# balkce/beamform

Hardware: AMD Instinct MI355X
Metric: stft_frames_per_sec (higher is better)
Workload: dtype f64; 1 GPU; das 8-mic 1024-pt (hop 512), 65536-frame batch per GPU, 1 stream(s), planar input resident in HBM; frames_per_gpu=65536, frames_fed_per_gpu=65536, mics=8, fft=1024, hop=512, streams=1, layout=planar, gather=n/a, parallelism=independent batches x1, input=uniform noise in [-0.5, 0.5), settle_launches_before_warmup=416, forward_transforms_per_frame_pair=6

## Files before the change

beamform_amd/csrc/das_f64_w64.hip:

```cpp
#include <hip/hip_runtime.h>

#include <cstdlib>
#include <cstring>
#include <type_traits>

#include "launch_trace.hpp"
#include "das_f64_plan.hpp"
#include "pipeline_kernels.hpp"
#include "w64_f64_dev.hpp"

namespace bf {

namespace {

constexpr int kBlock = 512;
constexpr int kWaves = kBlock / 64;
constexpr int kHop = 512;
constexpr int kTwD = 2 * (1024 + 4 * kTw2RowW64Rot);
constexpr int oTw = 0;
constexpr int oPlane = kTwD;
constexpr int oGain = oPlane + kWaves * kPlaneD;
constexpr int oCross = oGain + 4 * 2048;
constexpr int oFlag = oCross + 512;
constexpr int kWinRow = 18;
constexpr int oWin = oFlag + 8;
constexpr int kLdsD = oWin + 64 * kWinRow;

typedef volatile __attribute__((address_space(3))) int *lds_flag_t;

template <int LAYOUT>
__global__ __launch_bounds__(kBlock) void das_f64_w64_kernel(DasF64Args a, int frames_per_chunk, int chunks_per_stream) {
    __shared__ __attribute__((aligned(16))) double lds[kLdsD];
    const cx<double> *s_tw1 = reinterpret_cast<const cx<double> *>(lds + oTw);
    const cx<double> *s_tw2 = s_tw1 + 1024;
    const cx<double> *s_gain = reinterpret_cast<const cx<double> *>(lds + oGain);
    float *s_cross = reinterpret_cast<float *>(lds + oCross);
    lds_flag_t s_ready = (lds_flag_t)(lds + oFlag);
    lds_flag_t s_cons = s_ready + kWaves;

    const int tid = threadIdx.x, lane = tid & 63;
    const int w = __builtin_amdgcn_readfirstlane(tid >> 6);
    const int M = a.n_mics, NP = (M + 1) >> 1;
    double *plane = lds + oPlane + w * kPlaneD;
    double *wcol = plane + w64_col_rot(lane);
    double *row16 = plane + (lane & 15) * kRS + 16 * (lane >> 4);

    const int stream = blockIdx.x / chunks_per_stream;
    const long c_in_s = blockIdx.x - (long)stream * chunks_per_stream;
    const double *wrow = lds + oWin + lane * kWinRow;

    const long T0 = c_in_s * frames_per_chunk;
    long T1 = T0 + frames_per_chunk;
    if (T1 > a.n_frames) T1 = a.n_frames;
    const float *xs = a.x + (long)stream * a.stream_stride_x;
    const float *hs = a.hist + (long)stream * M * kHop;
    float *ys = a.y + (long)stream * a.n_frames * kHop;

    float na[16], nb[16];
    auto request = [&](long tt, int p) {
        const int ma = 2 * p, mb = (2 * p + 1 < M) ? 2 * p + 1 : ma;
        if (LAYOUT == 0) {
            const float *a1 = tt >= 1 ? xs + (long)ma * a.mic_stride + (tt - 1) * kHop : hs + ma * kHop;
            const float *b1 = tt >= 1 ? xs + (long)mb * a.mic_stride + (tt - 1) * kHop : hs + mb * kHop;
            const float *a2 = xs + (long)ma * a.mic_stride + tt * kHop;
            const float *b2 = xs + (long)mb * a.mic_stride + tt * kHop;
#pragma unroll
            for (int j = 0; j < 8; ++j) {
                na[j] = a1[(unsigned)(64 * j + lane)];
                nb[j] = b1[(unsigned)(64 * j + lane)];
                na[j + 8] = a2[(unsigned)(64 * j + lane)];
                nb[j + 8] = b2[(unsigned)(64 * j + lane)];
            }
        } else {
            const float *s1 = tt >= 1 ? xs + (tt - 1) * (long)kHop * M : hs;
            const float *s2 = xs + tt * (long)kHop * M;
            if ((M & 1) == 0) {
#pragma unroll
                for (int j = 0; j < 8; ++j) {
                    const float2 v1 = *reinterpret_cast<const float2 *>(s1 + (unsigned)((64 * j + lane) * M + ma));
                    const float2 v2 = *reinterpret_cast<const float2 *>(s2 + (unsigned)((64 * j + lane) * M + ma));
                    na[j] = v1.x;
                    nb[j] = v1.y;
                    na[j + 8] = v2.x;
                    nb[j + 8] = v2.y;
                }
            } else {
#pragma unroll
                for (int j = 0; j < 8; ++j) {
                    na[j] = s1[(unsigned)((64 * j + lane) * M + ma)];
                    nb[j] = s1[(unsigned)((64 * j + lane) * M + mb)];
                    na[j + 8] = s2[(unsigned)((64 * j + lane) * M + ma)];
                    nb[j + 8] = s2[(unsigned)((64 * j + lane) * M + mb)];
                }
            }
        }
    };

    const int n_iter = (int)((T1 - T0 + kWaves - 1) / kWaves);
    if (T0 + w < T1) request(T0 + w, 0);
    {
        const f64x2 *tw2 = a.tw, *g2 = a.gains;
        f64x2 *ltw = reinterpret_cast<f64x2 *>(lds + oTw), *lg = reinterpret_cast<f64x2 *>(lds + oGain);
#pragma unroll 4
        for (int i = tid; i < kTwD / 2; i += kBlock) ltw[i] = tw2[i];
#pragma unroll 8
        for (int i = tid; i < NP * 1024; i += kBlock) lg[i] = g2[i];
#pragma unroll 2
        for (int i = tid; i < 1024; i += kBlock) lds[oWin + (i & 63) * kWinRow + (i >> 6)] = a.win[i];
        if (tid < 2 * kWaves) s_ready[tid] = -2;
    }
    __syncthreads();
    for (int it = 0; it < n_iter; ++it) {
        const long t = T0 + (long)it * kWaves + w;
        if (t >= T1) break;

        double Sr[16], Si[16];
        for (int p = 0; p < NP; ++p) {
            double re[16], im[16];
            const bool b_ok = 2 * p + 1 < M;
#pragma unroll
            for (int j = 0; j < 8; ++j) {
                const double w0 = wrow[j], w1 = wrow[j + 8];
                const double t = (double)na[j] * w0, u = (double)na[j + 8];
                re[j] = fma(u, w1, t);
                re[j + 8] = fma(-u, w1, t);
            }
            if (b_ok) {
#pragma unroll
                for (int j = 0; j < 8; ++j) {
                    const double w0 = wrow[j], w1 = wrow[j + 8];
                    const double t = (double)nb[j] * w0, u = (double)nb[j + 8];
                    im[j] = fma(u, w1, t);
                    im[j + 8] = fma(-u, w1, t);
                }
            } else {
#pragma unroll
                for (int j = 0; j < 16; ++j) im[j] = 0.0;
            }
            {
                long tn = t;
                int pn = p + 1;
                if (pn == NP) {
                    pn = 0;
                    if (t + kWaves < T1) tn = t + kWaves;
                }
                request(tn, pn);
            }
            cx<double> tw[15];
            BF_STAGE();
            load_tw1<1, 9>(tw, s_tw1, lane);
            BF_STAGE();
            fft16_core<double, -1, true, 1>(re, im);
            BF_STAGE();
            load_tw1<9, 16>(tw, s_tw1, lane);
            BF_STAGE();
            mul_tw<false, 1, 9>(re, im, tw);
            BF_STAGE();
            mul_tw<false, 9, 16>(re, im, tw);
            if (p == 0 && it > 0 && w < kWaves - 1)
                while (s_cons[w] < (int)(t - kWaves)) __builtin_amdgcn_s_sleep(1);
            asm volatile("" ::: "memory");
            BF_STAGE();
            T1_fwd(re, im, wcol, row16);
            load_tw2<1, 9>(tw, s_tw2, lane);
            BF_STAGE();
            fft16_core<double, -1, true>(re, im);
            BF_STAGE();
            load_tw2<9, 16>(tw, s_tw2, lane);
            BF_STAGE();
            mul_tw<false, 1, 9>(re, im, tw);
            BF_STAGE();
            mul_tw<false, 9, 16>(re, im, tw);
            BF_STAGE();
            w64_T2<true>(re, im);
            cx<double> g[16];
            const cx<double> *gp = s_gain + p * 1024 + lane;
            BF_STAGE();
#pragma unroll
            for (int r = 0; r < 8; ++r) g[r] = gp[64 * r];
            BF_STAGE();
            w64_fwd_p3<double>(re, im);
            BF_STAGE();
#pragma unroll
            for (int r = 8; r < 16; ++r) g[r] = gp[64 * r];
            BF_STAGE();
            if (p == 0) {
#pragma unroll
                for (int r = 0; r < 16; ++r) {
                    if (r == 8) BF_STAGE();
                    Sr[r] = fma(-g[r].y, im[r], g[r].x * re[r]);
                    Si[r] = fma(g[r].y, re[r], g[r].x * im[r]);
                }
            } else {
#pragma unroll
                for (int r = 0; r < 16; ++r) {
                    if (r == 8) BF_STAGE();
                    Sr[r] = fma(-g[r].y, im[r], fma(g[r].x, re[r], Sr[r]));
                    Si[r] = fma(g[r].y, re[r], fma(g[r].x, im[r], Si[r]));
                }
            }
        }
        cx<double> tw[15];
        BF_STAGE();
        load_tw2<1, 16>(tw, s_tw2, lane);
        BF_STAGE();
        w64_inv_p3<double>(Sr, Si);
        w64_T2<false>(Sr, Si);
        BF_STAGE();
        mul_tw<true, 1, 16>(Sr, Si, tw);
        BF_STAGE();
        load_tw1<1, 16>(tw, s_tw1, lane);
        BF_STAGE();
        fft16_core<double, +1, false>(Sr, Si);
        BF_STAGE();
        T1_inv(Sr, Si, row16, wcol);
        BF_STAGE();
        mul_tw<true, 1, 16>(Sr, Si, tw);
        fft16_core<double, +1, false>(Sr, Si);

        float o[16];
#pragma unroll
        for (int j = 0; j < 16; ++j) {
            const float f = (float)Sr[j];
            o[j] = (float)((double)f * wrow[j]);
        }
        const int pw = (w + kWaves - 1) & (kWaves - 1);
        if (t + 1 < T1) {
            float *area = (w < kWaves - 1) ? reinterpret_cast<float *>(plane) : s_cross + (it & 1) * kHop;
            if (w == kWaves - 1 && it >= 2)
                while (s_cons[w] < (int)(t - 2 * kWaves)) __builtin_amdgcn_s_sleep(1);
            asm volatile("" ::: "memory");
#pragma unroll
            for (int j = 0; j < 8; ++j) area[64 * j + lane] = o[j + 8];
            asm volatile("" ::: "memory");
            if (lane == 0) s_ready[w] = (int)t;
        }
        float *yo = ys + t * kHop;
        if (t == T0) {
            if (T0 == 0) {
                const float *ti = a.tail_in + (long)stream * kHop;
#pragma unroll
                for (int j = 0; j < 8; ++j) yo[(unsigned)(64 * j + lane)] = ti[(unsigned)(64 * j + lane)] + o[j];
            } else {
#pragma unroll
                for (int j = 0; j < 8; ++j) atomicAdd(yo + (unsigned)(64 * j + lane), o[j]);
            }
        } else {
            const float *parea = (pw < kWaves - 1) ? reinterpret_cast<const float *>(lds + oPlane + pw * kPlaneD) : s_cross + ((it + 1) & 1) * kHop;
            while (s_ready[pw] < (int)(t - 1)) __builtin_amdgcn_s_sleep(1);
            asm volatile("" ::: "memory");
            float prev[8];
#pragma unroll
            for (int j = 0; j < 8; ++j) prev[j] = parea[64 * j + lane];
            asm volatile("" ::: "memory");
            if (lane == 0) s_cons[pw] = (int)(t - 1);
#pragma unroll
            for (int j = 0; j < 8; ++j) yo[(unsigned)(64 * j + lane)] = prev[j] + o[j];
        }
        if (t == T1 - 1) {
            if (T1 < a.n_frames) {
                float *yn = ys + T1 * kHop;
#pragma unroll
                for (int j = 0; j < 8; ++j) atomicAdd(yn + (unsigned)(64 * j + lane), o[j + 8]);
            } else {
                float *to = a.tail_out + (long)stream * kHop;
#pragma unroll
                for (int j = 0; j < 8; ++j) to[(unsigned)(64 * j + lane)] = o[j + 8];
            }
        }
    }
}


#ifdef BF_PARK_PLAIN
#define BF_PARK_LD(p) (*(const volatile float *)(p))
#else
#define BF_PARK_LD(p) __builtin_nontemporal_load(p)
#endif
constexpr int kGRow = 65;
constexpr int kGMic = 8 * kGRow;
constexpr int kSlots = 64;
constexpr int kTwP = 2 * (960 + 4 * kTw2RowW64Rot);
constexpr int pTw = 0;
constexpr int pPlane = kTwP;
constexpr int pGain = pPlane + kWaves * kPlaneD;
constexpr int pFlag = pGain + 7 * kGMic * 2;
constexpr int kRingR = 32;
constexpr int kRingSlots = kRingR + kWaves;
constexpr int pRing = pFlag + (kSlots + 4) / 2;
constexpr int pWin = pRing + kRingR / 2;
constexpr int kLdsP = pWin + 64 * kWinRow;
static_assert(kLdsP * 8 <= 160 * 1024, "LDS");
static_assert((pGain & 1) == 0 && (pWin & 1) == 0, "16-byte alignment");


typedef volatile __attribute__((address_space(3))) int *lds_int_t;
typedef volatile __attribute__((address_space(3))) unsigned long long *lds_u64_t;
__device__ __forceinline__ int lds_fetch_add(lds_int_t p, int v, int lane) {
    int old = 0;
    if (lane == 0) old = __hip_atomic_fetch_add((__attribute__((address_space(3))) int *)p, v, __ATOMIC_RELAXED, __HIP_MEMORY_SCOPE_WORKGROUP);
    return __builtin_amdgcn_readfirstlane(old);
}
__device__ __forceinline__ unsigned long long lds_fetch_add64(lds_u64_t p, int lane) {
    unsigned long long old = 0;
    if (lane == 0) old = __hip_atomic_fetch_add((__attribute__((address_space(3))) unsigned long long *)p, 1ull, __ATOMIC_RELAXED, __HIP_MEMORY_SCOPE_WORKGROUP);
    const unsigned lo = (unsigned)__builtin_amdgcn_readfirstlane((int)(unsigned)old), hi = (unsigned)__builtin_amdgcn_readfirstlane((int)(unsigned)(old >> 32));
    return ((unsigned long long)hi << 32) | lo;
}
struct DasSched {
    const int4 *chunks;
    unsigned *counter;
    int n_chunks;
};
__device__ __forceinline__ unsigned long long pack_work(unsigned vbase, int chunk, int pairs, int next) {
    return ((unsigned long long)(vbase & 0xFFFFFFu) << 40) | ((unsigned long long)(unsigned)chunk << 20) | ((unsigned long long)(unsigned)pairs << 10) | (unsigned)next;
}
struct PairWork {
    int4 d;
    int pos;
    int len;
    unsigned u;
    bool have;
};
__device__ __forceinline__ int4 load_chunk(const int4 *chunks, int k) {
    const int4 d = chunks[k];
    return int4{__builtin_amdgcn_readfirstlane(d.x), __builtin_amdgcn_readfirstlane(d.y), __builtin_amdgcn_readfirstlane(d.z), k};
}
__device__ __forceinline__ PairWork draw_pair(lds_u64_t work, const DasSched &sc, int lane, const int4 held) {
    PairWork r;
    r.have = false;
    r.d = int4{0, 0, 0, 0};
    r.pos = r.len = 0;
    r.u = 0;
    for (;;) {
        const unsigned long long old = lds_fetch_add64(work, lane);
        const int pos = (int)(old & 1023u), len = (int)((old >> 10) & 1023u), k = (int)((old >> 20) & 0xFFFFFu);
        const unsigned vb = (unsigned)(old >> 40);
        if (k == kChunkEnd) return r;
        if (pos < len) {
            if (k == held.w) r.d = held;
            else r.d = load_chunk(sc.chunks, k);
            r.pos = pos; r.len = len; r.u = vb + (unsigned)pos; r.have = true;
            return r;
        }
        if (pos == len) {
            unsigned k2 = 0;
            if (lane == 0) k2 = __hip_atomic_fetch_add(sc.counter, 1u, __ATOMIC_RELAXED, __HIP_MEMORY_SCOPE_AGENT);
            k2 = (unsigned)__builtin_amdgcn_readfirstlane((int)k2);
            if (k2 >= (unsigned)sc.n_chunks) {
                if (lane == 0) *work = pack_work(vb + (unsigned)len, kChunkEnd, 0, 0);
                return r;
            }
            r.d = load_chunk(sc.chunks, (int)k2);
            r.len = (r.d.z + 1) >> 1;
            r.pos = 0; r.u = vb + (unsigned)len; r.have = true;
            if (lane == 0) *work = pack_work(r.u, (int)k2, r.len, 1);
            return r;
        }
        while ((int)((*work >> 20) & 0xFFFFFu) == k) __builtin_amdgcn_s_sleep(2);
    }
}
__device__ __forceinline__ int claim_boundary(lds_int_t st, unsigned b, int lane) {
    const int base = 4 * (int)(b / kSlots);
    while (st[b & (kSlots - 1)] < base) __builtin_amdgcn_s_sleep(1);
    return lds_fetch_add(st + (b & (kSlots - 1)), 1, lane) - base;
}
__device__ __forceinline__ void publish_boundary(lds_int_t st, unsigned b, int lane) { (void)lds_fetch_add(st + (b & (kSlots - 1)), 2, lane); }
__device__ __forceinline__ void skip_boundary(lds_int_t st, unsigned b, int lane) {
    const int base = 4 * (int)(b / kSlots);
    while (st[b & (kSlots - 1)] < base) __builtin_amdgcn_s_sleep(1);
    (void)lds_fetch_add(st + (b & (kSlots - 1)), 4, lane);
}
__device__ __forceinline__ void await_boundary(lds_int_t st, unsigned b) {
    while (st[b & (kSlots - 1)] - 4 * (int)(b / kSlots) < 3) __builtin_amdgcn_s_sleep(1);
}

#ifdef BF_W64_STATS
__device__ unsigned long long g_stats[256 * 8 * 5];
#define BF_STATS_DECL unsigned long long st_[5] = {0, 0, 0, 0, 0}; const unsigned long long st_t0_ = __builtin_amdgcn_s_memrealtime()
#define BF_STAT(i) (++st_[i])
#define BF_STAT_WAIT_BEGIN const unsigned long long st_w0_ = __builtin_amdgcn_s_memrealtime()
#define BF_STAT_WAIT_END st_[3] += __builtin_amdgcn_s_memrealtime() - st_w0_
#define BF_STATS_FLUSH do { st_[4] = __builtin_amdgcn_s_memrealtime() - st_t0_; if (lane == 0 && blockIdx.x < 256) for (int i_ = 0; i_ < 5; ++i_) g_stats[(blockIdx.x * 8 + w) * 5 + i_] = st_[i_]; } while (0)
#else
#define BF_STATS_DECL
#define BF_STAT(i) ((void)0)
#define BF_STAT_WAIT_BEGIN
#define BF_STAT_WAIT_END
#define BF_STATS_FLUSH
#endif
#ifdef BF_W64_STAMPS
__device__ unsigned long long g_stamps[256 * 8 * 64];
#define BF_STAMP(slot) do { if (lane == 0 && blockIdx.x < 256 && (slot) < 64) g_stamps[(blockIdx.x * 8 + w) * 64 + (slot)] = __builtin_amdgcn_s_memrealtime(); } while (0)
#else
#define BF_STAMP(slot) do { } while (0)
#endif

typedef float il_f4 __attribute__((ext_vector_type(4)));
template <int LG>
__device__ __forceinline__ void il_tile_through_plane(const il_f4 (&v)[4], float *tile, float *dst, int t, int lane) {
    constexpr int M = 1 << LG, R1 = LG == 3 ? 10 : M + 1, spt = 1024 >> LG;
    asm volatile("" : "+v"(lane)::"memory");
#pragma unroll
    for (int i = 0; i < 4; ++i) {
#pragma unroll
        for (int c = 0; c < 4; ++c) {
            const int e = 256 * i + 4 * lane + c;
            tile[(e >> LG) * R1 + (e & (M - 1))] = v[i][c];
        }
    }
    asm volatile("" ::: "memory");
    __builtin_amdgcn_wave_barrier();
#pragma unroll
    for (int j = 0; j < 4; ++j) {
        const int mic = lane & (M - 1), q4 = (lane >> LG) + (64 >> LG) * j;
        il_f4 o;
#pragma unroll
        for (int c = 0; c < 4; ++c) o[c] = tile[(4 * q4 + c) * R1 + mic];
        reinterpret_cast<il_f4 *>(dst + mic * kHop + t * spt)[q4] = o;
    }
    asm volatile("" ::: "memory");
    __builtin_amdgcn_wave_barrier();
}

template <int LAYOUT>
__device__ __forceinline__ void das_f64_pair_body(const DasF64Args &a, const DasSched &sc) {
    __shared__ __attribute__((aligned(16))) double lds[kLdsP];
    const cx<double> *s_tw1 = reinterpret_cast<const cx<double> *>(lds + pTw) - 64;
    const cx<double> *s_tw2 = reinterpret_cast<const cx<double> *>(lds + pTw) + 960;
    const cx<double> *s_gain = reinterpret_cast<const cx<double> *>(lds + pGain);
    lds_int_t s_state = (lds_int_t)(lds + pFlag);
    lds_u64_t s_work = (lds_u64_t)(lds + pFlag + kSlots / 2);
    lds_int_t s_ring = (lds_int_t)(lds + pRing);
    (void)s_ring;

    const int tid = threadIdx.x, lane = tid & 63;
    const int w = __builtin_amdgcn_readfirstlane(tid >> 6);
    const int M = a.n_mics;
    double *plane = lds + pPlane + w * kPlaneD;
    double *wcol = plane + w64_col_rot(lane);
    double *row16 = plane + (lane & 15) * kRS + 16 * (lane >> 4);
    const double *wrow = lds + pWin + lane * kWinRow;
    typedef double cxa __attribute__((ext_vector_type(2)));
    typedef const __attribute__((address_space(3))) cxa *lds_gain_t;
    unsigned gd0 = (unsigned)(size_t)(lds_gain_t)(s_gain + lane);
    asm volatile("" : "+v"(gd0));
    gd0 &= ~15u;
    const unsigned g_mirror = 2u * (unsigned)(size_t)(lds_gain_t)s_gain + 1024u;

    float n0[8], n1[8], n2[8];
#ifndef BF_PAIR_NT
#define BF_PAIR_NT 0
#endif
    auto request = [&](const float *h0, const float *h1, const float *h2) {
#pragma unroll
        for (int j = 0; j < 8; ++j) {
            n0[j] = (BF_PAIR_NT & 2) ? __builtin_nontemporal_load(h0 + (unsigned)(64 * j + lane)) : h0[(unsigned)(64 * j + lane)];
            n1[j] = (BF_PAIR_NT & 1) ? __builtin_nontemporal_load(h1 + (unsigned)(64 * j + lane)) : h1[(unsigned)(64 * j + lane)];
            n2[j] = (BF_PAIR_NT & 4) ? __builtin_nontemporal_load(h2 + (unsigned)(64 * j + lane)) : h2[(unsigned)(64 * j + lane)];
        }
    };
    auto request_pair_mic = [&](int stream, long tA, int m) {
        const float *h1 = a.x + (long)stream * a.stream_stride_x + (long)m * a.mic_stride + tA * kHop;
        const float *h0 = tA >= 1 ? h1 - kHop : a.hist + ((long)stream * M + m) * kHop;
        const float *h2 = tA + 1 < a.n_frames ? h1 + kHop : h1;
        request(h0, h1, h2);
    };
    float q0[8], q1[8], q2[8];
    const double inv_m = 1.0 / (double)M;
    float e0[8], e1[8], e2[8];
    const int NT = a.n_tr, XM = a.extra_mic;
    auto request_extra = [&](bool on, int stream, long tA) {
        if (!on) {
#pragma unroll
            for (int j = 0; j < 8; ++j) e0[j] = e1[j] = e2[j] = 0.f;
            return;
        }
        const float *h1 = a.x + (long)stream * a.stream_stride_x + (long)XM * a.mic_stride + tA * kHop;
        const float *h0 = tA >= 1 ? h1 - kHop : a.hist + ((long)stream * M + XM) * kHop;
        const float *h2 = tA + 1 < a.n_frames ? h1 + kHop : h1;
#pragma unroll
        for (int j = 0; j < 8; ++j) {
            e0[j] = h0[(unsigned)(64 * j + lane)];
            e1[j] = h1[(unsigned)(64 * j + lane)];
            e2[j] = h2[(unsigned)(64 * j + lane)];
        }
    };

    struct RingHops { const float *h, *a, *b; };
    typedef float f4 __attribute__((ext_vector_type(4)));
    const int lgM = 31 - __builtin_clz((unsigned)M);
    float *ringb = LAYOUT == 1 ? a.ring + (size_t)blockIdx.x * kRingSlots * M * kHop : nullptr;
    auto ring_slot = [&](unsigned j) { return ringb + (size_t)(j & (kRingR - 1)) * M * kHop; };
    auto il_load2 = [&](const float *src, int unit, f4 (&v)[2][4]) {
        const f4 *s4 = reinterpret_cast<const f4 *>(src);
#pragma unroll
        for (int tt = 0; tt < 2; ++tt) {
            const int t = 2 * unit + tt;
            if (2 * t < M) {
#pragma unroll
                for (int i = 0; i < 4; ++i) v[tt][i] = s4[t * 256 + i * 64 + lane];
            } else {
#pragma unroll
                for (int i = 0; i < 4; ++i) v[tt][i] = f4{0.f, 0.f, 0.f, 0.f};
            }
        }
    };
    auto il_store2 = [&](const f4 (&v)[2][4], float *dst, int unit) {
        float *tile = reinterpret_cast<float *>(plane);
#pragma unroll
        for (int tt = 0; tt < 2; ++tt) {
            const int t = 2 * unit + tt;
            if (2 * t < M) {
                if (lgM == 3) il_tile_through_plane<3>(v[tt], tile, dst, t, lane);
                else if (lgM == 2) il_tile_through_plane<2>(v[tt], tile, dst, t, lane);
                else il_tile_through_plane<1>(v[tt], tile, dst, t, lane);
            }
        }
    };
    auto prepare_pair = [&](const PairWork &pw) {
        RingHops r;
        const unsigned u2 = 2u * pw.u;
        const int sA = (int)(u2 & (kRingR - 1)), gen4 = 4 * (int)(u2 / kRingR);
        float *dA = ring_slot(u2), *dB = ring_slot(u2 + 1), *dH = ringb + (size_t)(kRingR + w) * M * kHop;
        const long tA = pw.d.y + 2L * pw.pos;
        const float *xs = a.x + (long)pw.d.x * a.stream_stride_x;
        while (s_ring[sA] < gen4 || s_ring[sA + 1] < gen4) __builtin_amdgcn_s_sleep(1);
        f4 v0[2][4], v1[2][4];
        const bool two = tA + 1 < a.n_frames, first = pw.pos == 0, wide = M > 4;
        const float *srcA = xs + tA * (long)kHop * M, *srcB = srcA + (long)kHop * M;
        const float *srcH = tA >= 1 ? srcA - (long)kHop * M : a.hist + (long)pw.d.x * M * kHop;
        il_load2(srcA, 0, v0);
        if (wide) il_load2(srcA, 1, v1);
        il_store2(v0, dA, 0);
        if (two) il_load2(srcB, 0, v0);
        if (wide) il_store2(v1, dA, 1);
        if (two && wide) il_load2(srcB, 1, v1);
        if (two) il_store2(v0, dB, 0);
        if (first) il_load2(srcH, 0, v0);
        if (two && wide) il_store2(v1, dB, 1);
        if (first && wide) il_load2(srcH, 1, v1);
        if (first) il_store2(v0, dH, 0);
        if (first && wide) il_store2(v1, dH, 1);
        __builtin_amdgcn_fence(__ATOMIC_RELEASE, "workgroup");
        (void)lds_fetch_add(s_ring + sA, 2, lane);
        (void)lds_fetch_add(s_ring + sA + 1, 2, lane);
        r.a = dA;
        r.b = two ? dB : dA;
        r.h = dH;
        if (!first) {
            const unsigned jp = u2 - 1;
            const int sP = (int)(jp & (kRingR - 1)), genp = 4 * (int)(jp / kRingR);
            while (s_ring[sP] - genp < 2) __builtin_amdgcn_s_sleep(1);
            r.h = ring_slot(jp);
        }
        __builtin_amdgcn_fence(__ATOMIC_ACQUIRE, "workgroup");
        return r;
    };
    auto release_pair = [&](const PairWork &pw, bool has_t) {
        const unsigned u2 = 2u * pw.u;
        (void)lds_fetch_add(s_ring + (u2 & (kRingR - 1)), 2, lane);
        (void)lds_fetch_add(s_ring + ((u2 + 1) & (kRingR - 1)), has_t ? 1 : 2, lane);
        if (pw.pos > 0) (void)lds_fetch_add(s_ring + ((u2 - 1) & (kRingR - 1)), 1, lane);
    };
    auto request_ring_mic = [&](const RingHops &r, int m) { request(r.h + m * kHop, r.a + m * kHop, r.b + m * kHop); };
    auto request_ring_extra = [&](bool on, const RingHops &r) {
        if (!on) {
#pragma unroll
            for (int j = 0; j < 8; ++j) e0[j] = e1[j] = e2[j] = 0.f;
            return;
        }
#pragma unroll
        for (int j = 0; j < 8; ++j) {
            e0[j] = r.h[XM * kHop + (unsigned)(64 * j + lane)];
            e1[j] = r.a[XM * kHop + (unsigned)(64 * j + lane)];
            e2[j] = r.b[XM * kHop + (unsigned)(64 * j + lane)];
        }
    };
    RingHops curR{nullptr, nullptr, nullptr};
    (void)curR;

    BF_STAMP(0);
#ifdef BF_W64_STAMPS
    if (lane == 0 && blockIdx.x < 256) g_stamps[(blockIdx.x * 8 + w) * 64 + 59] = __builtin_amdgcn_s_memtime();
#endif
    PairWork cur;
    cur.d = load_chunk(sc.chunks, (int)blockIdx.x);
    cur.len = (cur.d.z + 1) >> 1;
    const int n_static = cur.len < kWaves ? cur.len : kWaves;
    cur.pos = w;
    cur.u = (unsigned)w;
    cur.have = w < n_static;
    if (LAYOUT == 0 && cur.have) {
        request_pair_mic(cur.d.x, cur.d.y + 2L * w, a.slot_mic[0]);
        request_extra(XM >= 0, cur.d.x, cur.d.y + 2L * w);
    } else {
        request_extra(false, 0, 0);
    }
    {
        const f64x2 *tw2 = a.tw + 64;
        f64x2 *ltw = reinterpret_cast<f64x2 *>(lds + pTw), *lg = reinterpret_cast<f64x2 *>(lds + pGain);
#pragma unroll 4
        for (int i = tid; i < kTwP / 2; i += kBlock) ltw[i] = tw2[i];
        for (int k = 0; k < NT; ++k) {
            const f64x2 *g2 = a.gains_mic + a.slot_mic[k] * kGMic;
#pragma unroll 2
            for (int i = tid; i < kGMic; i += kBlock) lg[k * kGMic + i] = g2[i];
        }
#pragma unroll 2
        for (int i = tid; i < 1024; i += kBlock) lds[pWin + (i & 63) * kWinRow + (i >> 6)] = a.win[i];
        if (tid < kSlots) s_state[tid] = 0;
        if (tid < kRingR) s_ring[tid] = 0;
        if (tid == 0) *s_work = pack_work(0u, (int)blockIdx.x, cur.len, n_static);
    }
    __syncthreads();
    BF_STAMP(1);
    BF_STATS_DECL;
    int it = 0;
    if (!cur.have) {
        cur = draw_pair(s_work, sc, lane, cur.d);
        if (LAYOUT == 0 && cur.have) {
            request_pair_mic(cur.d.x, cur.d.y + 2L * cur.pos, a.slot_mic[0]);
            request_extra(XM >= 0, cur.d.x, cur.d.y + 2L * cur.pos);
        }
    }
    while (cur.have) {
        if constexpr (LAYOUT == 1) {
            curR = prepare_pair(cur);
            request_ring_mic(curR, a.slot_mic[0]);
            request_ring_extra(XM >= 0, curR);
        }
        const int stream = cur.d.x;
        const long T0 = cur.d.y, T1 = T0 + cur.d.z;
        const long tA = T0 + 2L * cur.pos;
        const bool pair = tA + 1 < T1;
        const long tL = pair ? tA + 1 : tA;
        const unsigned u = cur.u;
        const bool has_t = cur.pos + 1 < cur.len, has_h = cur.pos > 0;
        float *ys = a.y + (long)stream * a.n_frames * kHop;
        PairWork nxt;
        nxt.have = false;
        const float *hp0 = a.x + (long)stream * a.stream_stride_x + tA * kHop;
        const float *hist0 = a.hist + (long)stream * M * kHop;
        const bool first_hop = tA < 1, last_hop = !(tA + 1 < a.n_frames);
        (void)hp0; (void)hist0; (void)first_hop; (void)last_hop;

        double Sr[16], Si[16];
        auto one_mic = [&](const int k, auto first_tag) {
            constexpr bool FIRST = decltype(first_tag)::value;
            double re[16], im[16];
#ifndef BF_PAIR_NO_VMWAIT
            if constexpr (!FIRST) __builtin_amdgcn_s_waitcnt(0x0F70);
#endif
            if (FIRST && XM >= 0) {
#pragma unroll
                for (int j = 0; j < 8; ++j) {
                    const double w0 = wrow[j], w1 = wrow[j + 8];
                    const double c = (double)n1[j] + (double)e1[j];
                    const double t = ((double)n0[j] + (double)e0[j]) * w0;
                    re[j] = fma(c, w1, t);
                    re[j + 8] = fma(-c, w1, t);
                    const double t2 = c * w0, u2 = (double)n2[j] + (double)e2[j];
                    im[j] = fma(u2, w1, t2);
                    im[j + 8] = fma(-u2, w1, t2);
                }
            } else {
#pragma unroll
                for (int j = 0; j < 8; ++j) {
                    const double w0 = wrow[j], w1 = wrow[j + 8];
                    const double c = (double)n1[j];
                    const double t = (double)n0[j] * w0;
                    re[j] = fma(c, w1, t);
                    re[j + 8] = fma(-c, w1, t);
                    const double t2 = c * w0, u2 = (double)n2[j];
                    im[j] = fma(u2, w1, t2);
                    im[j + 8] = fma(-u2, w1, t2);
                }
            }
            if (__builtin_expect(!pair, 0)) {
#ifndef BF_PAIR_CNDMASK
                asm volatile("" ::: "memory");
#endif
#pragma unroll
                for (int j = 0; j < 16; ++j) im[j] = 0.0;
            }
            if (k + 1 < NT) {
                if constexpr (LAYOUT == 1) request_ring_mic(curR, a.slot_mic[k + 1]);
                else request_pair_mic(stream, tA, a.slot_mic[k + 1]);
            } else {
                nxt = draw_pair(s_work, sc, lane, cur.d);
                if constexpr (LAYOUT == 0) {
                    if (nxt.have) request_pair_mic(nxt.d.x, nxt.d.y + 2L * nxt.pos, a.slot_mic[0]);
                    else request_pair_mic(stream, tA, a.slot_mic[0]);
                }
            }
            cx<double> tw[15];
            BF_STAGE();
            load_tw1<1, 9>(tw, s_tw1, lane);
            BF_STAGE();
            fft16_core<double, -1, true, 1>(re, im);
            BF_STAGE();
            load_tw1<9, 16>(tw, s_tw1, lane);
            BF_STAGE();
            mul_tw<false, 1, 9>(re, im, tw);
            BF_STAGE();
            mul_tw<false, 9, 16>(re, im, tw);
            BF_STAGE();
            T1_fwd(re, im, wcol, row16);
            load_tw2<1, 9>(tw, s_tw2, lane);
            BF_STAGE();
            fft16_core<double, -1, true>(re, im);
            BF_STAGE();
            load_tw2<9, 16>(tw, s_tw2, lane);
            BF_STAGE();
            mul_tw<false, 1, 9>(re, im, tw);
            BF_STAGE();
            mul_tw<false, 9, 16>(re, im, tw);
            BF_STAGE();
            w64_T2_any<true>(re, im, row16 - 16 * (lane >> 4), lane >> 4);
            cxa g[16];
            const lds_gain_t gd = (lds_gain_t)(size_t)(gd0 + (unsigned)(k * kGMic * 16));
            const lds_gain_t gm = (lds_gain_t)(size_t)((g_mirror + (unsigned)(2 * k * kGMic * 16)) - (gd0 + (unsigned)(k * kGMic * 16)));
            BF_STAGE();
#pragma unroll
            for (int r = 0; r < 8; ++r)
                g[r] = (r & 3) < 2 ? gd[(2 * (r >> 2) + (r & 3)) * kGRow] : gm[(2 * (3 - (r >> 2)) + 3 - (r & 3)) * kGRow];
            BF_STAGE();
            w64_fwd_p3<double>(re, im);
            BF_STAGE();
#pragma unroll
            for (int r = 8; r < 16; ++r)
                g[r] = (r & 3) < 2 ? gd[(2 * (r >> 2) + (r & 3)) * kGRow] : gm[(2 * (3 - (r >> 2)) + 3 - (r & 3)) * kGRow];
            BF_STAGE();
#pragma unroll
            for (int r = 0; r < 16; ++r) {
                if (r == 8) BF_STAGE();
                const double gx = g[r].x, gy = (r & 3) < 2 ? g[r].y : -g[r].y;
                if constexpr (FIRST) {
                    Sr[r] = fma(-gy, im[r], gx * re[r]);
                    Si[r] = fma(gy, re[r], gx * im[r]);
                } else {
                    Sr[r] = fma(-gy, im[r], fma(gx, re[r], Sr[r]));
                    Si[r] = fma(gy, re[r], fma(gx, im[r], Si[r]));
                }
            }
        };
        one_mic(0, std::true_type{});
        for (int k = 1; k < NT; ++k) one_mic(k, std::false_type{});
        float *yo = ys + tA * kHop;
        cx<double> tw[15];
        BF_STAGE();
        {
            const float *h0 = LAYOUT == 1 ? curR.h : (first_hop ? hist0 : hp0 - kHop), *h1 = LAYOUT == 1 ? curR.a : hp0;
            const float *h2 = LAYOUT == 1 ? curR.b : (last_hop ? hp0 : hp0 + kHop);
#pragma unroll
            for (int j = 0; j < 8; ++j) {
                q0[j] = h0[(unsigned)(64 * j + lane)];
                q1[j] = h1[(unsigned)(64 * j + lane)];
                q2[j] = h2[(unsigned)(64 * j + lane)];
            }
            if constexpr (LAYOUT == 0) request_extra(XM >= 0 && nxt.have, nxt.d.x, nxt.d.y + 2L * nxt.pos);
        }
        BF_STAGE();
        load_tw2<1, 16>(tw, s_tw2, lane);
        BF_STAGE();
        w64_inv_p3<double>(Sr, Si);
        w64_T2_any<false>(Sr, Si, row16 - 16 * (lane >> 4), lane >> 4);
        BF_STAGE();
        mul_tw<true, 1, 16>(Sr, Si, tw);
        BF_STAGE();
        load_tw1<1, 16>(tw, s_tw1, lane);
        BF_STAGE();
        fft16_core<double, +1, false>(Sr, Si);
        BF_STAGE();
        T1_inv(Sr, Si, row16, wcol);
        BF_STAGE();
        mul_tw<true, 1, 16>(Sr, Si, tw);
        fft16_core<double, +1, false>(Sr, Si);

#pragma unroll
        for (int j = 0; j < 8; ++j) {
            const double w0 = wrow[j], w1 = wrow[j + 8];
            const double c = (double)q1[j];
            Sr[j] = fma((double)q0[j] * w0, inv_m, Sr[j]);
            Sr[j + 8] = fma(c * w1, inv_m, Sr[j + 8]);
            Si[j] = fma(c * w0, inv_m, Si[j]);
            Si[j + 8] = fma((double)q2[j] * w1, inv_m, Si[j + 8]);
        }
        float oA[16], tl[8];
        if (pair) {
#pragma unroll
            for (int j = 0; j < 8; ++j) {
                const float f1 = (float)Si[j + 8];
                tl[j] = (float)((double)f1 * wrow[j + 8]);
            }
        } else {
#pragma unroll
            for (int j = 0; j < 8; ++j) {
                const float f1 = (float)Sr[j + 8];
                tl[j] = (float)((double)f1 * wrow[j + 8]);
            }
        }
        float *yn = ys + (tL + 1) * kHop;
        int oT = -1, oH = -1;
        if (has_t) {
            oT = claim_boundary(s_state, u, lane);
            if (oT == 0) {
#pragma unroll
                for (int j = 0; j < 8; ++j) yn[(unsigned)(64 * j + lane)] = tl[j];
            }
        } else {
            skip_boundary(s_state, u, lane);
        }
#pragma unroll
        for (int j = 0; j < 16; ++j) {
            const float f = (float)Sr[j];
            oA[j] = (float)((double)f * wrow[j]);
        }
        if (pair) {
            float *y1 = ys + (tA + 1) * kHop;
#pragma unroll
            for (int j = 0; j < 8; ++j) {
                const float f0 = (float)Si[j];
                const float b0 = (float)((double)f0 * wrow[j]);
                y1[(unsigned)(64 * j + lane)] = oA[j + 8] + b0;
            }
        }
        if (has_h) {
            oH = claim_boundary(s_state, u - 1, lane);
            if (oH == 0) {
#pragma unroll
                for (int j = 0; j < 8; ++j) yo[(unsigned)(64 * j + lane)] = oA[j];
            }
        } else if (T0 == 0) {
            const float *ti = a.tail_in + (long)stream * kHop;
#pragma unroll
            for (int j = 0; j < 8; ++j) yo[(unsigned)(64 * j + lane)] = ti[(unsigned)(64 * j + lane)] + oA[j];
        } else {
#pragma unroll
            for (int j = 0; j < 8; ++j) atomicAdd(yo + (unsigned)(64 * j + lane), oA[j]);
        }
        if (oT == 0 || oH == 0) {
            __builtin_amdgcn_fence(__ATOMIC_RELEASE, "workgroup");
            if (oT == 0) publish_boundary(s_state, u, lane);
            if (oH == 0) publish_boundary(s_state, u - 1, lane);
        }
        if (oT > 0) {
            BF_STAT(2);
            BF_STAT_WAIT_BEGIN;
            await_boundary(s_state, u);
            BF_STAT_WAIT_END;
            __builtin_amdgcn_fence(__ATOMIC_ACQUIRE, "workgroup");
            float o[8];
#pragma unroll
            for (int j = 0; j < 8; ++j) o[j] = BF_PARK_LD(yn + (unsigned)(64 * j + lane));
#pragma unroll
            for (int j = 0; j < 8; ++j) yn[(unsigned)(64 * j + lane)] = tl[j] + o[j];
        } else {
            BF_STAT(0);
        }
        if (oH > 0) {
            BF_STAT(2);
            BF_STAT_WAIT_BEGIN;
            await_boundary(s_state, u - 1);
            BF_STAT_WAIT_END;
            __builtin_amdgcn_fence(__ATOMIC_ACQUIRE, "workgroup");
            float o[8];
#pragma unroll
            for (int j = 0; j < 8; ++j) o[j] = BF_PARK_LD(yo + (unsigned)(64 * j + lane));
#pragma unroll
            for (int j = 0; j < 8; ++j) yo[(unsigned)(64 * j + lane)] = o[j] + oA[j];
        } else {
            BF_STAT(1);
        }
        if (!has_t) {
            if (T1 < a.n_frames) {
                float *ynx = ys + T1 * kHop;
#pragma unroll
                for (int j = 0; j < 8; ++j) atomicAdd(ynx + (unsigned)(64 * j + lane), tl[j]);
            } else {
                float *to = a.tail_out + (long)stream * kHop;
#pragma unroll
                for (int j = 0; j < 8; ++j) to[(unsigned)(64 * j + lane)] = tl[j];
                if (a.hist_out != nullptr) {
                    float *ho = a.hist_out + (long)stream * M * kHop;
                    const float *xs = a.x + (long)stream * a.stream_stride_x;
                    for (int m = 0; m < M; ++m) {
                        const float *xl = xs + (long)m * a.mic_stride + tL * kHop;
#pragma unroll
                        for (int j = 0; j < 8; ++j) ho[m * kHop + 64 * j + lane] = xl[(unsigned)(64 * j + lane)];
                    }
                }
            }
        }
        if constexpr (LAYOUT == 1) {
            asm volatile("" ::: "memory");
            release_pair(cur, has_t);
        }
        cur = nxt;
        ++it;
    }
    BF_STATS_FLUSH;
#ifdef BF_W64_STAMPS
    if (lane == 0 && blockIdx.x < 256) {
        g_stamps[(blockIdx.x * 8 + w) * 64 + 63] = __builtin_amdgcn_s_memrealtime();
        g_stamps[(blockIdx.x * 8 + w) * 64 + 60] = __builtin_amdgcn_s_memtime();
        g_stamps[(blockIdx.x * 8 + w) * 64 + 62] = (unsigned long long)it;
        g_stamps[(blockIdx.x * 8 + w) * 64 + 61] = (unsigned long long)__builtin_amdgcn_s_getreg(((4 - 1) << 11) | (0 << 6) | 20);
    }
#endif
    (void)it;
}

__global__ __launch_bounds__(kBlock) void das_f64_pair_kernel(DasF64Args a, DasSched sc) { das_f64_pair_body<0>(a, sc); }
__global__ __launch_bounds__(kBlock) void das_f64_ring_kernel(DasF64Args a, DasSched sc) { das_f64_pair_body<1>(a, sc); }

constexpr int kSchedPerBlock = 8;
__global__ __launch_bounds__(32 * kSchedPerBlock) void das_f64_sched_kernel(DasSchedPlan p, int4 *chunks, unsigned *counter, float *y, long n_frames, int n_streams) {
    const int k = blockIdx.x * kSchedPerBlock + (int)(threadIdx.x >> 5), l = (int)(threadIdx.x & 31);
    if (k >= p.n_chunks) return;
    int stream;
    long t0, n;
    das_f64_chunk(p, n_frames, n_streams, k, &stream, &t0, &n);
    if (l == 0) {
        chunks[k] = int4{stream, (int)t0, (int)n, 0};
        if (k == 0) *counter = (unsigned)p.grid;
    }
    if (t0 > 0) {
        float4 *h = reinterpret_cast<float4 *>(y + ((long)stream * n_frames + t0) * kHop);
        for (int i = l; i < kHop / 4; i += 32) h[i] = float4{0.f, 0.f, 0.f, 0.f};
    }
}

__global__ __launch_bounds__(256) void interleaved_to_planar_kernel(const float *x, float *out, long tiles_per_stream, int M, long in_stream_stride,
                                                                    long out_mic_stride, long out_stream_stride) {
    __shared__ float s_t[256 * 9];
    const int tid = threadIdx.x;
    const long s = blockIdx.x / tiles_per_stream, tile = blockIdx.x - s * tiles_per_stream;
    const float4 *src = reinterpret_cast<const float4 *>(x + s * in_stream_stride + tile * 256 * M);
    const int R = M + 1;
    for (int i = tid; i < 64 * M; i += 256) {
        const float4 v = src[i];
        const int e = 4 * i;
        s_t[(e / M) * R + e % M] = v.x;
        s_t[((e + 1) / M) * R + (e + 1) % M] = v.y;
        s_t[((e + 2) / M) * R + (e + 2) % M] = v.z;
        s_t[((e + 3) / M) * R + (e + 3) % M] = v.w;
    }
    __syncthreads();
    float *dst = out + s * out_stream_stride + tile * 256;
    for (int j = tid; j < 64 * M; j += 256) {
        const int m = j >> 6, q = j & 63;
        const float4 v{s_t[(4 * q) * R + m], s_t[(4 * q + 1) * R + m], s_t[(4 * q + 2) * R + m], s_t[(4 * q + 3) * R + m]};
        reinterpret_cast<float4 *>(dst + (long)m * out_mic_stride)[q] = v;
    }
}

}

static bool ring_mics(int m) { return m == 2 || m == 4 || m == 8; }
static bool use_pair_kernel(const DasF64Args &a) {
    if (!(a.gains_mic != nullptr && a.sched_ws != nullptr && a.mic0_unit != 0 && a.n_mics >= 2 && a.n_tr >= 1)) return false;
    if (a.layout == 0) return true;
    return a.ring != nullptr && ring_mics(a.n_mics) && a.hist_out == nullptr;
}
size_t das_f64_ring_bytes(int n_mics, int n_cus) {
    return ring_mics(n_mics) ? (size_t)n_cus * kRingSlots * n_mics * kHop * sizeof(float) : 0;
}

bool das_f64_writes_hist(const DasF64Args &a) { return use_pair_kernel(a) && a.hist_out != nullptr; }

constexpr size_t kSchedCounterBytes = 256;
size_t das_f64_sched_ws_bytes() { return kSchedCounterBytes + (size_t)kSchedMaxChunks * sizeof(int4); }

static void das_f64_w64_runs(const DasF64Args &a, int n_cus, long *fpc, long *cps) {
    const long step = kWaves;
    long runs = (long)n_cus / a.n_streams;
    if (runs < 1) runs = 1;
    long f = (a.n_frames + runs - 1) / runs;
    f = ((f + step - 1) / step) * step;
    *fpc = f;
    *cps = (a.n_frames + f - 1) / f;
}

hipError_t prepare_das_f64_w64(const DasF64Args &a, int n_cus, hipStream_t s) {
    if (a.n_mics > 8) return hipErrorNotSupported;
    if (use_pair_kernel(a)) {
        if (a.sched_ws_bytes < das_f64_sched_ws_bytes() || (long)a.n_streams * ((a.n_frames + 1) / 2) >= (1L << 31)) return hipErrorNotSupported;
        const DasSchedPlan p = das_f64_plan(a.n_frames, a.n_streams, n_cus, getenv("BF_DAS_F64_SCHED"));
        if (p.n_chunks < 1 || p.n_chunks > kSchedMaxChunks) return hipErrorNotSupported;
        unsigned *counter = reinterpret_cast<unsigned *>(a.sched_ws);
        int4 *chunks = reinterpret_cast<int4 *>(reinterpret_cast<char *>(a.sched_ws) + kSchedCounterBytes);
        BF_LAUNCH(das_f64_sched_kernel, dim3((unsigned)((p.n_chunks + kSchedPerBlock - 1) / kSchedPerBlock)), dim3(32 * kSchedPerBlock), 0, s, p, chunks, counter, a.y, a.n_frames, a.n_streams);
        return hipGetLastError();
    }
    if (a.layout == 0) return hipErrorNotSupported;
    long fpc, cps;
    das_f64_w64_runs(a, n_cus, &fpc, &cps);
    if (cps > 1)
        for (int st = 0; st < a.n_streams; ++st) {
            hipError_t e = hipMemset2DAsync(a.y + ((long)st * a.n_frames + fpc) * kHop, (size_t)fpc * kHop * sizeof(float), 0,
                                            kHop * sizeof(float), (size_t)cps - 1, s);
            if (e != hipSuccess) return e;
        }
    return hipSuccess;
}

hipError_t launch_interleaved_to_planar(const float *x, float *out, long n, int n_mics, int n_streams, hipStream_t s) {
    if (n_mics < 1 || n_mics > 8 || (n & 255) != 0) return hipErrorNotSupported;
    const long tiles = n / 256;
    BF_LAUNCH(interleaved_to_planar_kernel, dim3((unsigned)(tiles * n_streams)), dim3(256), 0, s, x, out, tiles, n_mics, (long)n_mics * n, n, (long)n_mics * n);
    return hipGetLastError();
}

hipError_t launch_das_f64_w64(const DasF64Args &a, int n_cus, hipStream_t s) {
    if (a.n_mics > 8) return hipErrorNotSupported;
    if (use_pair_kernel(a)) {
        const DasSchedPlan p = das_f64_plan(a.n_frames, a.n_streams, n_cus, getenv("BF_DAS_F64_SCHED"));
        DasSched sc;
        sc.counter = reinterpret_cast<unsigned *>(a.sched_ws);
        sc.chunks = reinterpret_cast<const int4 *>(reinterpret_cast<char *>(a.sched_ws) + kSchedCounterBytes);
        sc.n_chunks = p.n_chunks;
        if (a.layout == 0) {
            BF_LAUNCH(das_f64_pair_kernel, dim3((unsigned)p.grid), dim3(kBlock), 0, s, a, sc);
        } else {
            if (a.ring_bytes < das_f64_ring_bytes(a.n_mics, p.grid)) return hipErrorNotSupported;
            BF_LAUNCH(das_f64_ring_kernel, dim3((unsigned)p.grid), dim3(kBlock), 0, s, a, sc);
        }
        return hipGetLastError();
    }
    long fpc, cps;
    das_f64_w64_runs(a, n_cus, &fpc, &cps);
    if (a.layout == 0) return hipErrorNotSupported;
    BF_LAUNCH(das_f64_w64_kernel<1>, dim3((unsigned)(cps * a.n_streams)), dim3(kBlock), 0, s, a, (int)fpc, (int)cps);
    return hipGetLastError();
}

}

#ifdef BF_W64_STATS
extern "C" int bf_dbg_stats(unsigned long long *host) {
    return (int)hipMemcpyFromSymbol(host, HIP_SYMBOL(bf::g_stats), sizeof(unsigned long long) * 256 * 8 * 5);
}
#endif
#ifdef BF_W64_STAMPS
extern "C" int bf_dbg_stamps(unsigned long long *host) {
    return (int)hipMemcpyFromSymbol(host, HIP_SYMBOL(bf::g_stamps), sizeof(unsigned long long) * 256 * 8 * 64);
}
#endif
```

Measured before the change: 137.2 million frames/s.

## Park overlap-add boundary hops in spare LDS slots instead of global memory

The first wave to claim a frame-boundary hop now writes its partial overlap-add segment into a free LDS park slot, tracked by a bitmask, instead of global memory. The slot number is encoded in the per-boundary state word so the second wave reads the partial from LDS, adds, and frees the slot. This replaces the global write, workgroup release/acquire fences and nontemporal global reload with LDS traffic and a waitcnt. It falls back to the old global path when no slot is free, at the cost of more LDS per block (possible occupancy loss) and a more complex state protocol.

```diff
diff --git a/beamform_amd/csrc/das_f64_w64.hip b/beamform_amd/csrc/das_f64_w64.hip
--- a/beamform_amd/csrc/das_f64_w64.hip
+++ b/beamform_amd/csrc/das_f64_w64.hip
@@ -291,7 +291,13 @@
 constexpr int pWin = pRing + kRingR / 2;
 constexpr int kLdsP = pWin + 64 * kWinRow;
 static_assert(kLdsP * 8 <= 160 * 1024, "LDS");
-static_assert((pGain & 1) == 0 && (pWin & 1) == 0, "16-byte alignment");
+constexpr int kParkD = kHop / 2;
+constexpr int kParkFree = (160 * 1024 - kLdsP * 8) / (kParkD * 8);
+constexpr int kParkSlots = kParkFree < 15 ? kParkFree : 15;
+constexpr int pPark = kLdsP;
+constexpr int kLdsAll = pPark + kParkSlots * kParkD;
+static_assert(kLdsAll * 8 <= 160 * 1024, "LDS");
+static_assert((pGain & 1) == 0 && (pWin & 1) == 0 && (pPark & 1) == 0, "16-byte alignment");
 
 
 typedef volatile __attribute__((address_space(3))) int *lds_int_t;
@@ -311,6 +317,7 @@
     const int4 *chunks;
     unsigned *counter;
     int n_chunks;
+    int park_slots;
 };
 __device__ __forceinline__ unsigned long long pack_work(unsigned vbase, int chunk, int pairs, int next) {
     return ((unsigned long long)(vbase & 0xFFFFFFu) << 40) | ((unsigned long long)(unsigned)chunk << 20) | ((unsigned long long)(unsigned)pairs << 10) | (unsigned)next;
@@ -360,33 +367,61 @@
         while ((int)((*work >> 20) & 0xFFFFFu) == k) __builtin_amdgcn_s_sleep(2);
     }
 }
+constexpr int kLife = 64, kInHop = 63;
+static_assert(2 + 4 * (kParkSlots - 1) + 2 < kInHop, "the park slot number fits the state word");
 __device__ __forceinline__ int claim_boundary(lds_int_t st, unsigned b, int lane) {
-    const int base = 4 * (int)(b / kSlots);
+    const int base = kLife * (int)(b / kSlots);
     while (st[b & (kSlots - 1)] < base) __builtin_amdgcn_s_sleep(1);
     return lds_fetch_add(st + (b & (kSlots - 1)), 1, lane) - base;
 }
-__device__ __forceinline__ void publish_boundary(lds_int_t st, unsigned b, int lane) { (void)lds_fetch_add(st + (b & (kSlots - 1)), 2, lane); }
+__device__ __forceinline__ void publish_boundary(lds_int_t st, unsigned b, int slot, int lane) {
+    (void)lds_fetch_add(st + (b & (kSlots - 1)), slot >= 0 ? 2 + 4 * slot : kLife - 2, lane);
+}
 __device__ __forceinline__ void skip_boundary(lds_int_t st, unsigned b, int lane) {
-    const int base = 4 * (int)(b / kSlots);
+    const int base = kLife * (int)(b / kSlots);
     while (st[b & (kSlots - 1)] < base) __builtin_amdgcn_s_sleep(1);
-    (void)lds_fetch_add(st + (b & (kSlots - 1)), 4, lane);
-}
-__device__ __forceinline__ void await_boundary(lds_int_t st, unsigned b) {
-    while (st[b & (kSlots - 1)] - 4 * (int)(b / kSlots) < 3) __builtin_amdgcn_s_sleep(1);
+    (void)lds_fetch_add(st + (b & (kSlots - 1)), kLife, lane);
+}
+__device__ __forceinline__ int await_boundary(lds_int_t st, unsigned b) {
+    const int base = kLife * (int)(b / kSlots);
+    int v;
+    while ((v = st[b & (kSlots - 1)] - base) < 3) __builtin_amdgcn_s_sleep(1);
+    return __builtin_amdgcn_readfirstlane(v);
+}
+__device__ __forceinline__ int take_park_slot(lds_int_t free_bits, int lane) {
+    int s = -1;
+    if (lane == 0) {
+        const unsigned m = (unsigned)*free_bits;
+        if (m != 0u) {
+            const unsigned bit = m & (0u - m);
+            const unsigned old = __hip_atomic_fetch_and((__attribute__((address_space(3))) unsigned *)free_bits, ~bit, __ATOMIC_RELAXED, __HIP_MEMORY_SCOPE_WORKGROUP);
+            if (old & bit) s = __builtin_ctz(bit);
+        }
+    }
+    return __builtin_amdgcn_readfirstlane(s);
+}
+__device__ __forceinline__ void consume_boundary(lds_int_t st, lds_int_t free_bits, unsigned b, int slot, int lane) {
+    if (lane == 0) (void)__hip_atomic_fetch_or((__attribute__((address_space(3))) unsigned *)free_bits, 1u << slot, __ATOMIC_RELAXED, __HIP_MEMORY_SCOPE_WORKGROUP);
+    (void)lds_fetch_add(st + (b & (kSlots - 1)), kLife - 4 - 4 * slot, lane);
 }
 
 #ifdef BF_W64_STATS
-__device__ unsigned long long g_stats[256 * 8 * 5];
-#define BF_STATS_DECL unsigned long long st_[5] = {0, 0, 0, 0, 0}; const unsigned long long st_t0_ = __builtin_amdgcn_s_memrealtime()
+constexpr int kStats = 8;
+__device__ unsigned long long g_stats[256 * 8 * kStats];
+#define BF_STATS_DECL unsigned long long st_[kStats] = {0, 0, 0, 0, 0, 0, 0, 0}; const unsigned long long st_t0_ = __builtin_amdgcn_s_memrealtime()
 #define BF_STAT(i) (++st_[i])
 #define BF_STAT_WAIT_BEGIN const unsigned long long st_w0_ = __builtin_amdgcn_s_memrealtime()
 #define BF_STAT_WAIT_END st_[3] += __builtin_amdgcn_s_memrealtime() - st_w0_
-#define BF_STATS_FLUSH do { st_[4] = __builtin_amdgcn_s_memrealtime() - st_t0_; if (lane == 0 && blockIdx.x < 256) for (int i_ = 0; i_ < 5; ++i_) g_stats[(blockIdx.x * 8 + w) * 5 + i_] = st_[i_]; } while (0)
+#define BF_STAT_ORDER_BEGIN const unsigned long long st_f0_ = __builtin_amdgcn_s_memrealtime()
+#define BF_STAT_ORDER_END st_[7] += __builtin_amdgcn_s_memrealtime() - st_f0_
+#define BF_STATS_FLUSH do { st_[4] = __builtin_amdgcn_s_memrealtime() - st_t0_; if (lane == 0 && blockIdx.x < 256) for (int i_ = 0; i_ < kStats; ++i_) g_stats[(blockIdx.x * 8 + w) * kStats + i_] = st_[i_]; } while (0)
 #else
 #define BF_STATS_DECL
 #define BF_STAT(i) ((void)0)
 #define BF_STAT_WAIT_BEGIN
 #define BF_STAT_WAIT_END
+#define BF_STAT_ORDER_BEGIN
+#define BF_STAT_ORDER_END
 #define BF_STATS_FLUSH
 #endif
 #ifdef BF_W64_STAMPS
@@ -425,12 +460,14 @@
 
 template <int LAYOUT>
 __device__ __forceinline__ void das_f64_pair_body(const DasF64Args &a, const DasSched &sc) {
-    __shared__ __attribute__((aligned(16))) double lds[kLdsP];
+    __shared__ __attribute__((aligned(16))) double lds[kLdsAll];
     const cx<double> *s_tw1 = reinterpret_cast<const cx<double> *>(lds + pTw) - 64;
     const cx<double> *s_tw2 = reinterpret_cast<const cx<double> *>(lds + pTw) + 960;
     const cx<double> *s_gain = reinterpret_cast<const cx<double> *>(lds + pGain);
     lds_int_t s_state = (lds_int_t)(lds + pFlag);
     lds_u64_t s_work = (lds_u64_t)(lds + pFlag + kSlots / 2);
+    lds_int_t s_free = s_state + kSlots + 2;
+    float *s_park = reinterpret_cast<float *>(lds + pPark);
     lds_int_t s_ring = (lds_int_t)(lds + pRing);
     (void)s_ring;
 
@@ -612,6 +649,7 @@
         if (tid < kSlots) s_state[tid] = 0;
         if (tid < kRingR) s_ring[tid] = 0;
         if (tid == 0) *s_work = pack_work(0u, (int)blockIdx.x, cur.len, n_static);
+        if (tid == 0) *s_free = (int)((1u << sc.park_slots) - 1u);
     }
     __syncthreads();
     BF_STAMP(1);
@@ -803,11 +841,21 @@
         }
         float *yn = ys + (tL + 1) * kHop;
         int oT = -1, oH = -1;
+        int sT = -1, sH = -1;
         if (has_t) {
             oT = claim_boundary(s_state, u, lane);
             if (oT == 0) {
-#pragma unroll
-                for (int j = 0; j < 8; ++j) yn[(unsigned)(64 * j + lane)] = tl[j];
+                sT = take_park_slot(s_free, lane);
+                if (sT >= 0) {
+                    BF_STAT(5);
+                    float *pk = s_park + sT * kHop;
+#pragma unroll
+                    for (int j = 0; j < 8; ++j) pk[64 * j + lane] = tl[j];
+                } else {
+                    BF_STAT(6);
+#pragma unroll
+                    for (int j = 0; j < 8; ++j) yn[(unsigned)(64 * j + lane)] = tl[j];
+                }
             }
         } else {
             skip_boundary(s_state, u, lane);
@@ -829,8 +877,17 @@
         if (has_h) {
             oH = claim_boundary(s_state, u - 1, lane);
             if (oH == 0) {
-#pragma unroll
-                for (int j = 0; j < 8; ++j) yo[(unsigned)(64 * j + lane)] = oA[j];
+                sH = take_park_slot(s_free, lane);
+                if (sH >= 0) {
+                    BF_STAT(5);
+                    float *pk = s_park + sH * kHop;
+#pragma unroll
+                    for (int j = 0; j < 8; ++j) pk[64 * j + lane] = oA[j];
+                } else {
+                    BF_STAT(6);
+#pragma unroll
+                    for (int j = 0; j < 8; ++j) yo[(unsigned)(64 * j + lane)] = oA[j];
+                }
             }
         } else if (T0 == 0) {
             const float *ti = a.tail_in + (long)stream * kHop;
@@ -841,35 +898,67 @@
             for (int j = 0; j < 8; ++j) atomicAdd(yo + (unsigned)(64 * j + lane), oA[j]);
         }
         if (oT == 0 || oH == 0) {
-            __builtin_amdgcn_fence(__ATOMIC_RELEASE, "workgroup");
-            if (oT == 0) publish_boundary(s_state, u, lane);
-            if (oH == 0) publish_boundary(s_state, u - 1, lane);
+            BF_STAT_ORDER_BEGIN;
+            if ((oT == 0 && sT < 0) || (oH == 0 && sH < 0)) {
+                __builtin_amdgcn_fence(__ATOMIC_RELEASE, "workgroup");
+            } else {
+                asm volatile("" ::: "memory");
+                __builtin_amdgcn_s_waitcnt(0xC07F);
+                asm volatile("" ::: "memory");
+            }
+            BF_STAT_ORDER_END;
+            if (oT == 0) publish_boundary(s_state, u, sT, lane);
+            if (oH == 0) publish_boundary(s_state, u - 1, sH, lane);
         }
         if (oT > 0) {
             BF_STAT(2);
             BF_STAT_WAIT_BEGIN;
-            await_boundary(s_state, u);
+            const int v = await_boundary(s_state, u);
             BF_STAT_WAIT_END;
-            __builtin_amdgcn_fence(__ATOMIC_ACQUIRE, "workgroup");
             float o[8];
-#pragma unroll
-            for (int j = 0; j < 8; ++j) o[j] = BF_PARK_LD(yn + (unsigned)(64 * j + lane));
-#pragma unroll
-            for (int j = 0; j < 8; ++j) yn[(unsigned)(64 * j + lane)] = tl[j] + o[j];
+            if (v >= kInHop) {
+                __builtin_amdgcn_fence(__ATOMIC_ACQUIRE, "workgroup");
+#pragma unroll
+                for (int j = 0; j < 8; ++j) o[j] = BF_PARK_LD(yn + (unsigned)(64 * j + lane));
+#pragma unroll
+                for (int j = 0; j < 8; ++j) yn[(unsigned)(64 * j + lane)] = tl[j] + o[j];
+            } else {
+                const int ps = (v - 3) >> 2;
+                const float *pk = s_park + ps * kHop;
+                asm volatile("" ::: "memory");
+#pragma unroll
+                for (int j = 0; j < 8; ++j) o[j] = pk[64 * j + lane];
+#pragma unroll
+                for (int j = 0; j < 8; ++j) yn[(unsigned)(64 * j + lane)] = tl[j] + o[j];
+                asm volatile("" ::: "memory");
+                consume_boundary(s_state, s_free, u, ps, lane);
+            }
         } else {
             BF_STAT(0);
         }
         if (oH > 0) {
             BF_STAT(2);
             BF_STAT_WAIT_BEGIN;
-            await_boundary(s_state, u - 1);
+            const int v = await_boundary(s_state, u - 1);
             BF_STAT_WAIT_END;
-            __builtin_amdgcn_fence(__ATOMIC_ACQUIRE, "workgroup");
             float o[8];
-#pragma unroll
-            for (int j = 0; j < 8; ++j) o[j] = BF_PARK_LD(yo + (unsigned)(64 * j + lane));
-#pragma unroll
-            for (int j = 0; j < 8; ++j) yo[(unsigned)(64 * j + lane)] = o[j] + oA[j];
+            if (v >= kInHop) {
+                __builtin_amdgcn_fence(__ATOMIC_ACQUIRE, "workgroup");
+#pragma unroll
+                for (int j = 0; j < 8; ++j) o[j] = BF_PARK_LD(yo + (unsigned)(64 * j + lane));
+#pragma unroll
+                for (int j = 0; j < 8; ++j) yo[(unsigned)(64 * j + lane)] = o[j] + oA[j];
+            } else {
+                const int ps = (v - 3) >> 2;
+                const float *pk = s_park + ps * kHop;
+                asm volatile("" ::: "memory");
+#pragma unroll
+                for (int j = 0; j < 8; ++j) o[j] = pk[64 * j + lane];
+#pragma unroll
+                for (int j = 0; j < 8; ++j) yo[(unsigned)(64 * j + lane)] = o[j] + oA[j];
+                asm volatile("" ::: "memory");
+                consume_boundary(s_state, s_free, u - 1, ps, lane);
+            }
         } else {
             BF_STAT(1);
         }
@@ -1013,6 +1102,16 @@
     return hipGetLastError();
 }
 
+static int das_f64_park_slots() {
+    static const int n = [] {
+        const char *e = getenv("BF_DAS_PARK_SLOTS");
+        if (e == nullptr || *e == 0) return kParkSlots;
+        const int v = atoi(e);
+        return v < 0 ? 0 : (v > kParkSlots ? kParkSlots : v);
+    }();
+    return n;
+}
+
 hipError_t launch_das_f64_w64(const DasF64Args &a, int n_cus, hipStream_t s) {
     if (a.n_mics > 8) return hipErrorNotSupported;
     if (use_pair_kernel(a)) {
@@ -1021,6 +1120,7 @@
         sc.counter = reinterpret_cast<unsigned *>(a.sched_ws);
         sc.chunks = reinterpret_cast<const int4 *>(reinterpret_cast<char *>(a.sched_ws) + kSchedCounterBytes);
         sc.n_chunks = p.n_chunks;
+        sc.park_slots = das_f64_park_slots();
         if (a.layout == 0) {
             BF_LAUNCH(das_f64_pair_kernel, dim3((unsigned)p.grid), dim3(kBlock), 0, s, a, sc);
         } else {
@@ -1040,7 +1140,7 @@
 
 #ifdef BF_W64_STATS
 extern "C" int bf_dbg_stats(unsigned long long *host) {
-    return (int)hipMemcpyFromSymbol(host, HIP_SYMBOL(bf::g_stats), sizeof(unsigned long long) * 256 * 8 * 5);
+    return (int)hipMemcpyFromSymbol(host, HIP_SYMBOL(bf::g_stats), sizeof(unsigned long long) * 256 * 8 * bf::kStats);
 }
 #endif
 #ifdef BF_W64_STAMPS
```

Result: no change. 138.0 million frames/s (median of 6 runs) (+0.6%).
